# google/yggdrasil-decision-forests

Hardware: NVIDIA H100
Metric: GBT boosting iters/sec, 10M rows x 200 num feats (higher is better)
Workload: dtype int64 fixed-point sums (q24 gradients), f64 split scores

## Files before the change

include/ygg_b200.h:

```cpp
#ifndef YGG_B200_H_
#define YGG_B200_H_

#include <stdint.h>

#ifdef __cplusplus
extern "C" {
#endif

#define YGG_ABI_VERSION 3

enum ygg_status {
  YGG_OK = 0,
  YGG_ERR_INVALID_ARGUMENT = 1,
  YGG_ERR_NO_DEVICE = 2,
  YGG_ERR_CUDA = 3,
  YGG_ERR_UNIMPLEMENTED = 4,
  YGG_ERR_CANCELLED = 5,
  YGG_ERR_IO = 6
};

enum ygg_loss {
  YGG_LOSS_BINOMIAL_LOG_LIKELIHOOD = 0,
  YGG_LOSS_SQUARED_ERROR = 1,
  YGG_LOSS_MULTINOMIAL_LOG_LIKELIHOOD = 2
// ... 145 lines not shown
int ygg_gbt_tie_stats(ygg_gbt* h, int64_t* renamed, int64_t* unresolved);
int ygg_gbt_set_tie_rng_position(ygg_gbt* h, uint64_t words);

int ygg_num_candidate_attributes(int32_t num_features, int32_t loss, int32_t num_candidate_attributes,
                                 float num_candidate_attributes_ratio, int32_t* k);
uint64_t ygg_candidate_key(uint32_t random_seed, int32_t tree, int32_t node, int32_t feature);
int ygg_gbt_set_candidate_sampling(ygg_gbt* h, int32_t num_candidate_attributes, float num_candidate_attributes_ratio);

int ygg_gbt_set_dart(ygg_gbt* h, float dropout_rate);
int ygg_gbt_get_dart_weights(ygg_gbt* h, float* out, int32_t capacity, int32_t* n);
int ygg_gbt_get_dart_dropped(ygg_gbt* h, int32_t iter, int32_t* out, int32_t capacity, int32_t* n);

int ygg_gbt_get_tree(ygg_gbt* h, int32_t iter, ygg_node* out, int32_t capacity, int32_t* n_nodes);
int ygg_gbt_get_category_set(ygg_gbt* h, int32_t iter, int32_t node, uint32_t* words, int32_t capacity, int32_t* n_words);
int ygg_gbt_train_loss(ygg_gbt* h, int32_t iter, float* loss, float* secondary);
int ygg_gbt_get_predictions(ygg_gbt* h, float* out, int64_t n);
int ygg_gbt_predict(ygg_gbt* h, const ygg_dataset* ds, float* out, int64_t n);

int ygg_gbt_set_predictions(ygg_gbt* h, const float* pred, int64_t n);

int ygg_tree_train_on_gradients(ygg_gbt* h, const float* gradients, const float* hessians,
                                ygg_node* out, int32_t capacity, int32_t* n_nodes);

enum ygg_hist_mode {
  YGG_HIST_ROOT_SUM = 0,
  YGG_HIST_PACKED = 1,
  YGG_HIST_SHARED = 2,
  YGG_HIST_HIST2 = 3,
  YGG_HIST_SEGMENTED = 4,
};
typedef struct ygg_hist_plan {
  int32_t mode;
  int32_t group;
  int32_t hist2_tiles;
  int32_t chunk_blocks;
  int32_t slot_window;
  int32_t grid;
} ygg_hist_plan;
int ygg_debug_hist_plan(const ygg_gbt* h, int32_t level, ygg_hist_plan* out);
int ygg_debug_level_histogram(ygg_gbt* h, int32_t level, const ygg_hist_plan* plan, const float* gradients,
                              const float* second, const int32_t* slot_of_row, int32_t n_slots, uint64_t* out_sum,
                              uint32_t* out_cnt, uint64_t* out_second, float* out_scales);

int ygg_debug_wide_histogram(ygg_gbt* h, int32_t n_slots, uint64_t* out_sum, uint32_t* out_cnt, uint64_t* out_second);

int ygg_debug_capture_candidates(ygg_gbt* h, int32_t enabled);
typedef struct ygg_level_node {
  int32_t node;
  int32_t candidate;
  int32_t derived;
  int32_t reserved;
  int64_t num_examples;
} ygg_level_node;
typedef struct ygg_candidate {
  int32_t found;
  float score;
  int32_t threshold_bin;
  int32_t lo, hi;
  int32_t num_pos_examples;
  float threshold_value;
  uint32_t cat_mask[8];
} ygg_candidate;
int ygg_debug_level_candidates(ygg_gbt* h, int32_t level, int32_t capacity, ygg_level_node* nodes, ygg_candidate* cands,
                               uint32_t* sets, int32_t set_words, int32_t* n_nodes, float* scales);
int ygg_debug_level_tried(ygg_gbt* h, int32_t level, int32_t capacity, uint8_t* tried, int32_t* first_node, int32_t* n_nodes);

int ygg_partition_rows(ygg_dataset* ds, const uint32_t* rows_in, int64_t n, int32_t feature,
// ... 14 lines not shown
```

yggdrasil-decision-forests_b200/_capi.py:

```python
import ctypes as C
import os

import numpy as np

from . import _build

_LIB = None


class YggError(RuntimeError):
    def __init__(self, code, msg):
        super().__init__(f"[ygg status {code}] {msg}")
        self.code = code


class GbtConfig(C.Structure):
    _fields_ = [
        ("abi_version", C.c_int32), ("loss", C.c_int32), ("num_trees", C.c_int32),
        ("shrinkage", C.c_float), ("max_depth", C.c_int32), ("min_examples", C.c_int32),
        ("in_split_min_examples_check", C.c_int32), ("use_hessian_gain", C.c_int32),
        ("l1_regularization", C.c_float), ("l2_regularization", C.c_float),
        ("l2_regularization_categorical", C.c_float), ("clamp_leaf_logit", C.c_float),
        ("hessian_split_score_subtract_parent", C.c_int32), ("random_seed", C.c_uint32),
        ("subsample", C.c_float), ("validation_ratio", C.c_float),
        ("sibling_subtraction", C.c_int32), ("early_stopping", C.c_int32),
        ("early_stopping_num_trees_look_ahead", C.c_int32), ("early_stopping_initial_iteration", C.c_int32),
        ("num_classes", C.c_int32), ("candidate_shuffle", C.c_int32), ("rng_words_consumed", C.c_uint32),
        ("split_jobs_draw_seeds", C.c_int32), ("growing_strategy", C.c_int32), ("max_num_nodes", C.c_int32),
        ("goss_alpha", C.c_float), ("goss_beta", C.c_float),
    ]


NODE_DTYPE = np.dtype([
    ("feature", "<i4"), ("threshold_bin", "<i4"), ("na_value", "<i4"), ("depth", "<i4"),
    ("neg_child", "<i4"), ("pos_child", "<i4"), ("split_score", "<f4"), ("leaf_value", "<f4"),
    ("num_examples", "<i8"), ("num_pos_examples", "<i8"), ("stat", "<f8", (3,)),
    ("condition_type", "<i4"), ("threshold_value", "<f4"), ("cat_mask", "<u4", (8,)),
])
assert NODE_DTYPE.itemsize == 112

FEATURE_DISCRETIZED_NUMERICAL = 0
FEATURE_CATEGORICAL = 1
FEATURE_NUMERICAL = 2

LEVEL_NODE_DTYPE = np.dtype([("node", "<i4"), ("candidate", "<i4"), ("derived", "<i4"), ("reserved", "<i4"),
                             ("num_examples", "<i8")])
assert LEVEL_NODE_DTYPE.itemsize == 24
CANDIDATE_DTYPE = np.dtype([("found", "<i4"), ("score", "<f4"), ("threshold_bin", "<i4"), ("lo", "<i4"), ("hi", "<i4"),
                            ("num_pos_examples", "<i4"), ("threshold_value", "<f4"), ("cat_mask", "<u4", (8,))])
assert CANDIDATE_DTYPE.itemsize == 60

HIST_ROOT_SUM, HIST_PACKED, HIST_SHARED, HIST2, HIST_SEGMENTED = 0, 1, 2, 3, 4


class HistPlan(C.Structure):
    _fields_ = [("mode", C.c_int32), ("group", C.c_int32), ("hist2_tiles", C.c_int32), ("chunk_blocks", C.c_int32),
                ("slot_window", C.c_int32), ("grid", C.c_int32)]

    def __repr__(self):
        return "HistPlan(%s)" % ", ".join("%s=%d" % (k, getattr(self, k)) for k, _ in self._fields_)

ALLGATHER_FN = C.CFUNCTYPE(C.c_int, C.c_void_p, C.c_void_p, C.c_void_p, C.c_int64, C.c_void_p)
ALLREDUCE_FN = C.CFUNCTYPE(C.c_int, C.c_void_p, C.c_void_p, C.c_int64, C.c_int32, C.c_int32, C.c_void_p)
REDUCESCATTER_FN = C.CFUNCTYPE(C.c_int, C.c_void_p, C.c_void_p, C.c_int64, C.c_int32, C.c_int32, C.c_void_p)

EXPORTS = [
    "ygg_abi_version", "ygg_last_error", "ygg_device_count", "ygg_dataset_create",
    "ygg_dataset_set_feature_types", "ygg_dataset_destroy", "ygg_dataset_num_rows", "ygg_dataset_num_features",
    "ygg_gbt_config_init", "ygg_gbt_create", "ygg_gbt_destroy", "ygg_gbt_set_labels_i32",
    "ygg_gbt_set_labels_f32", "ygg_gbt_set_weights_f32", "ygg_gbt_set_validation_weights_f32", "ygg_gbt_set_feature_shard", "ygg_gbt_set_row_shard", "ygg_gbt_set_row_shard_scatter", "ygg_feature_shard",
    "ygg_merge_shard_best", "ygg_gbt_initial_prediction",
    "ygg_gbt_train", "ygg_gbt_train_timed", "ygg_gbt_step", "ygg_gbt_sync", "ygg_gbt_num_trees", "ygg_gbt_get_tree",
    "ygg_gbt_train_loss", "ygg_gbt_get_predictions", "ygg_gbt_set_predictions", "ygg_gbt_predict",
    "ygg_tree_train_on_gradients", "ygg_debug_hist_plan", "ygg_debug_level_histogram", "ygg_partition_rows",
    "ygg_gbt_set_profiling", "ygg_gbt_get_profile", "ygg_gbt_save_ydf",
    "ygg_discretize_boundaries", "ygg_discretize_encode", "ygg_model_write_ydf",
    "ygg_validation_split_mask", "ygg_dataset_split_rows", "ygg_gbt_set_validation_i32",
    "ygg_gbt_set_validation_f32", "ygg_gbt_validation_loss", "ygg_gbt_num_iterations", "ygg_gbt_final_validation",
    "ygg_gen_discretized_boundaries", "ygg_dataset_builder_create", "ygg_dataset_builder_add_numerical",
    "ygg_dataset_builder_add_numerical_async", "ygg_dataset_builder_get_numerical",
    "ygg_dataset_builder_add_bins", "ygg_dataset_builder_finish", "ygg_dataset_builder_destroy",
    "ygg_dataset_get_bins", "ygg_dataset_set_bucket_values", "ygg_gbt_tie_stats", "ygg_gbt_set_tie_rng_position",
    "ygg_gbt_best_split_window_bytes", "ygg_gbt_set_best_split_window", "ygg_comm_window_create",
    "ygg_comm_unique_id", "ygg_comm_create", "ygg_comm_destroy", "ygg_comm_allreduce", "ygg_comm_allgather", "ygg_comm_reducescatter",
    "ygg_dataset_set_wide_column", "ygg_dataset_get_wide_column", "ygg_debug_wide_histogram",
    "ygg_dataset_set_wide_categorical_column", "ygg_gbt_get_category_set",
    "ygg_dataset_set_numerical_column", "ygg_dataset_get_numerical_column",
    "ygg_debug_capture_candidates", "ygg_debug_level_candidates",
    "ygg_num_candidate_attributes", "ygg_candidate_key", "ygg_gbt_set_candidate_sampling", "ygg_debug_level_tried",
    "ygg_gbt_set_dart", "ygg_gbt_get_dart_weights", "ygg_gbt_get_dart_dropped",
# ... 692 lines not shown
```

yggdrasil-decision-forests_b200/csrc/ygg_engine.cu:

```cuda
#include <algorithm>
#include <mutex>
#include <random>
#include <cmath>
#include <cstdarg>
#include <cstdio>
#include <cstdlib>
#include <cstring>
#include <limits>
#include <map>
#include <queue>
#include <string>
#include <thread>
#include <vector>

#include <cuda_runtime.h>
#include <cub/device/device_radix_sort.cuh>
#include <cub/device/device_scan.cuh>
#include <nvtx3/nvToolsExt.h>

#include "../../include/ygg_b200.h"
#include "ygg_internal.h"
#include "../../include/ygg_b200_model.h"
#include "ygg_kernels.cuh"
#include "ygg_wide.cuh"
#include "ygg_presort.cuh"
#include "ygg_hist_seg.cuh"

using namespace ygg;

namespace {

thread_local std::string g_last_error;

int set_error(int code, const char* fmt, ...) {
  char buf[1024];
  va_list ap;
  va_start(ap, fmt);
  vsnprintf(buf, sizeof(buf), fmt, ap);
  va_end(ap);
  g_last_error = buf;
  return code;
}

}

int ygg_set_error_msg(int code, const char* msg) { return set_error(code, "%s", msg); }

namespace {

#define YGG_CUDA(expr)                                                                          \
  do {                                                                                          \
    cudaError_t _e = (expr);                                                                    \
    if (_e != cudaSuccess)                                                                      \
      return set_error(YGG_ERR_CUDA, "%s failed: %s (%s:%d)", #expr, cudaGetErrorString(_e),    \
                       __FILE__, __LINE__);                                                     \
  } while (0)

#define YGG_RETURN_IF_ERROR(expr) \
// ... 29 lines not shown
  return YGG_OK;
}
template <typename T>
int dev_alloc_plain(T** p, size_t count) {
  YGG_CUDA(cudaMalloc(reinterpret_cast<void**>(p), std::max<size_t>(count, 1) * sizeof(T)));
  return YGG_OK;
}
inline void dev_free(void* p) {
  if (p != nullptr) cudaFreeAsync(p, nullptr);
}

struct ProfileSlot {
  double ms = 0;
  int64_t launches = 0;
};

}


struct LossRec {
  double loss_sum;
  unsigned long long correct;
};

enum ShardMode { kShardNone = 0, kShardFeatures = 1, kShardRows = 2 };

struct HistLaunch {
  int mode;
  int G, S;
  int chunk, grid;
  int window, passes;
  int FL, T;
  int SL;
};

struct ygg_gbt {
  ygg_dataset* ds = nullptr;
  ygg_gbt_config cfg{};
  cudaStream_t stream = nullptr;
  bool has_labels = false;
  uint8_t* d_label_u8 = nullptr;
  float* d_label_f32 = nullptr;
  float initial_prediction = 0.f;
  float* d_pred = nullptr;
  float* d_g = nullptr;
  float* d_h = nullptr;
  uint32_t* d_q24 = nullptr;
  uint32_t* d_hq24 = nullptr;
  uint2* d_act = nullptr;
  uint32_t* d_act_h = nullptr;
  int32_t* d_act_count = nullptr;
  int32_t* d_act_sub = nullptr;
  uint32_t* d_root_cnt = nullptr;
  bool root_cnt_valid = false;
  int n_blocks = 0;
  uint16_t* d_node_of_row = nullptr;
  DeviceState* d_st = nullptr;
  LevelDesc* d_levels = nullptr;
  Family* d_fam[2] = {nullptr, nullptr};
  int32_t* d_slot_node[2] = {nullptr, nullptr};
  NodeRec* d_nodes_all = nullptr;
  NodeRec* d_nodes_scratch = nullptr;
  int tree_capacity = 0;
  unsigned long long* d_hist_sum[2] = {nullptr, nullptr};
  uint32_t* d_hist_cnt[2] = {nullptr, nullptr};
  unsigned long long* d_hist_hsum[2] = {nullptr, nullptr};
// ... 309 lines not shown
  YGG_CUDA(cudaMemcpy(out_max, d_max, sizeof(uint32_t), cudaMemcpyDeviceToHost));
  return YGG_OK;
}

int raise_hist_smem_caps_once(int device) {
  static std::mutex mu;
  static std::vector<char> done;
  std::lock_guard<std::mutex> lock(mu);
  if (static_cast<int>(done.size()) <= device) done.resize(device + 1, 0);
  if (done[device]) return YGG_OK;
  size_t budget = 0;
  YGG_RETURN_IF_ERROR(hist_smem_budget(device, &budget));
  auto set_cap = [](size_t bytes) {
    return [bytes](auto kern) -> int {
      YGG_CUDA(cudaFuncSetAttribute(kern, cudaFuncAttributeMaxDynamicSharedMemorySize, static_cast<int>(bytes)));
      return YGG_OK;
    };
  };
  for (const bool hess : {false, true})
    for (const int mode : {kHistRootSum, kHistPacked, kHistShared})
      for (const bool multi : {false, true}) YGG_RETURN_IF_ERROR(for_hist_kernel(hess, mode, set_cap(budget), multi));
  const auto cap2 = set_cap(kHist2SmemBudget);
  YGG_RETURN_IF_ERROR(cap2(k_hist2<32, true>)); YGG_RETURN_IF_ERROR(cap2(k_hist2<32, false>));
  YGG_RETURN_IF_ERROR(cap2(k_hist2<16, true>)); YGG_RETURN_IF_ERROR(cap2(k_hist2<16, false>));
  YGG_RETURN_IF_ERROR(cap2(k_hist2<8, true>)); YGG_RETURN_IF_ERROR(cap2(k_hist2<8, false>));
  YGG_RETURN_IF_ERROR(set_cap(seg_smem_bytes(64))(k_hist_seg<32, 2>));
  YGG_RETURN_IF_ERROR(set_cap(seg_smem_bytes(32))(k_hist_seg<32, 1>));
  YGG_RETURN_IF_ERROR(set_cap(seg_smem_bytes(16))(k_hist_seg<16, 1>));
  YGG_RETURN_IF_ERROR(set_cap(seg_smem_bytes(8))(k_hist_seg<8, 1>));
  YGG_CUDA(cudaFuncSetAttribute(k_hist_seg<32, 2>, cudaFuncAttributePreferredSharedMemoryCarveout, cudaSharedmemCarveoutMaxShared));
  YGG_CUDA(cudaFuncSetAttribute(k_hist_seg<32, 1>, cudaFuncAttributePreferredSharedMemoryCarveout, cudaSharedmemCarveoutMaxShared));
  YGG_CUDA(cudaFuncSetAttribute(k_hist_seg<16, 1>, cudaFuncAttributePreferredSharedMemoryCarveout, cudaSharedmemCarveoutMaxShared));
  YGG_CUDA(cudaFuncSetAttribute(k_hist_seg<8, 1>, cudaFuncAttributePreferredSharedMemoryCarveout, cudaSharedmemCarveoutMaxShared));
  done[device] = 1;
  return YGG_OK;
}

int configure_launches(ygg_gbt* h) {
  (void)cudaGetLastError();
  const bool hh = hist_hess(h);
  size_t budget = 0;
  YGG_RETURN_IF_ERROR(hist_smem_budget(h->ds->device, &budget));
  YGG_RETURN_IF_ERROR(raise_hist_smem_caps_once(h->ds->device));
  const int f_count = h->hist_f_end - h->hist_f_begin;
  const int n_blocks = static_cast<int>(h->ds->n_pad / kBlockRows);
  const int kSubBlocks = sub_blocks_of(h);
  const double min_items = 1.0, min_items2 = 0.9;
  auto choose_chunk = [&](int n_fgroups, int grid, int step, double need) {
    const int max_c = std::max(step, kHistMaxChunkBlocks / step * step);
    const int min_chunks = std::max(1, (n_blocks + max_c - 1) / max_c);
    int best = max_c;
    double best_score = -1;
    for (int nc = min_chunks; nc <= std::max(min_chunks, n_blocks); nc++) {
      const int c = std::min(max_c, ((n_blocks + nc - 1) / nc + step - 1) / step * step);
      const int real_nc = (n_blocks + c - 1) / c;
      const double per_cta = static_cast<double>(real_nc) * n_fgroups / grid;
      if (per_cta > 8.0 && nc > min_chunks) break;
      const double fill = static_cast<double>(n_blocks) / (static_cast<double>(real_nc) * c);
      const double eff = per_cta / std::ceil(per_cta) * fill;
      const double score = eff + (per_cta >= need ? 0.08 : 0.0);
      if (score > best_score + 1e-9) { best_score = score; best = c; }
    }
    return best;
  };
  const int g_begin = h->hist_f_begin / 4, n_groups = (h->hist_f_end + 3) / 4 - g_begin;
  const char* env_hist2 = std::getenv("YGG_HIST2");
// ... 2 lines not shown
  for (int l = 0; l < h->num_levels; l++) {
    HistLaunch& pl = h->hist_plan[l];
    pl.mode = hh ? kHistShared : (l == 0 && !sampling(h)) ? kHistRootSum : kHistPacked;
    int S = level_slot_bound(h, l);
    pl.window = 0;
    pl.passes = 1;
    if (hist_smem_bytes(1, S, hh, pl.mode) > budget) {
      if (S > 254)
        return set_error(YGG_ERR_UNIMPLEMENTED, "max_depth=%d needs %d histogram slots at level %d; the active lists carry 8-bit slots",
                         h->cfg.max_depth, S, l);
      int s_pass = 1;
      while (hist_smem_bytes(1, 2 * s_pass + 1, hh, pl.mode) <= budget) s_pass *= 2;
      pl.window = s_pass;
      pl.passes = (S + s_pass - 1) / s_pass;
      S = s_pass + 1;
    }
    int G = 1;
    while (G < 8 && G < f_count && hist_smem_bytes(G + 1, S, hh, pl.mode) <= budget) G++;
    pl.G = G;
    pl.S = S;
    pl.grid = h->ds->num_sms;
    pl.FL = pl.T = 0;
    if (want_hist2 && !hh && S <= 2 && (l > 0 || pl.mode == kHistRootSum)) {
      int FL = 32;
      while (FL > 8 && FL / 2 >= 4 * n_groups) FL /= 2;
      int T = 2;
      if (hist2_smem_bytes(FL, S, T, l == 0) > kHist2SmemBudget) T = 1;
      if (hist2_smem_bytes(FL, S, T, l == 0) <= kHist2SmemBudget) { pl.FL = FL; pl.T = T; }
    }
    const bool packed = pl.mode == kHistPacked || (pl.FL > 0 && l > 0);
    const int n_fgroups = pl.FL > 0 ? (n_groups + pl.FL / 4 - 1) / (pl.FL / 4) : (f_count + G - 1) / G;
    pl.chunk = choose_chunk(n_fgroups, pl.grid, packed ? kSubBlocks : 1, pl.FL > 0 ? min_items2 : min_items);
    pl.SL = 0;
    khist_plan[l] = pl;
    const int S_level = level_slot_bound(h, l);
    if (!hh && l > 0 && pl.mode == kHistPacked && pl.FL == 0 && S_level >= seg_min_slots(f_count, h->ds->n)) {
      int SL = 32;
      while (SL > 8 && SL / 2 >= f_count) SL /= 2;
      pl.SL = SL;
      pl.G = 1;
      pl.S = S_level;
      pl.window = 0;
      pl.passes = 1;
      pl.grid = h->ds->num_sms * kSegMinBlocks;
      pl.chunk = std::min(std::max(kSubBlocks, kHistMaxChunkBlocks / kSubBlocks * kSubBlocks),
                          (n_blocks + kSubBlocks - 1) / kSubBlocks * kSubBlocks);
    }
  }
  {
    std::map<int, uint32_t> max_of_chunk;
    uint32_t* d_sub = nullptr;
    int status = YGG_OK;
    for (int l = 0; l < h->num_levels && status == YGG_OK; l++) {
      HistLaunch& pl = h->hist_plan[l];
      if (pl.mode != kHistPacked && (pl.FL == 0 || l == 0)) continue;
      int chunk = pl.chunk;
      while (chunk >= kSubBlocks) {
        auto it = max_of_chunk.find(chunk);
        if (it == max_of_chunk.end()) {
          uint32_t m = 0;
          status = chunk_max_count(h, chunk, &d_sub, &m);
          if (status != YGG_OK) break;
          it = max_of_chunk.emplace(chunk, m).first;
        }
        if (it->second <= kPackedMaxUpdates) break;
        const int smaller = static_cast<int>(static_cast<double>(chunk) * 0.9 * kPackedMaxUpdates / it->second) / kSubBlocks * kSubBlocks;
        const int next = std::min(smaller, chunk - kSubBlocks);
        chunk = (next < kSubBlocks && chunk > kSubBlocks) ? kSubBlocks : next;
      }
      if (chunk < kSubBlocks) {
        if (pl.SL > 0) pl = khist_plan[l];
        pl.mode = kHistShared;
        pl.FL = 0;
        pl.chunk = choose_chunk((f_count + pl.G - 1) / pl.G, pl.grid, 1, min_items);
      } else {
        pl.chunk = chunk;
      }
    }
    dev_free(d_sub);
    if (status != YGG_OK) return status;
  }
  h->part_smem_children = static_cast<int>((32 * 1024) / (kPartWords * sizeof(uint32_t)));
  return YGG_OK;
}

int allocate_wide_buffers(ygg_gbt* h) {
  const ygg_dataset* ds = h->ds;
  dev_free(h->d_wsum); dev_free(h->d_wcnt); dev_free(h->d_whsum);
  h->d_wsum = nullptr; h->d_wcnt = nullptr; h->d_whsum = nullptr;
  for (int i = 0; i < 2; i++) {
    dev_free(h->d_wnode_sum[i]); dev_free(h->d_wnode_cnt[i]); dev_free(h->d_wnode_hsum[i]);
    h->d_wnode_sum[i] = nullptr; h->d_wnode_cnt[i] = nullptr; h->d_wnode_hsum[i] = nullptr;
  }
  dev_free(h->d_wide_thr); dev_free(h->d_wide_feature); dev_free(h->d_wide_bins);
  h->d_wide_thr = nullptr; h->d_wide_feature = nullptr; h->d_wide_bins = nullptr;
  dev_free(h->d_wide_cat); dev_free(h->d_wide_na_bin); dev_free(h->d_wide_set); dev_free(h->d_sort_key); dev_free(h->d_sort_idx);
  h->d_wide_cat = nullptr; h->d_wide_na_bin = nullptr; h->d_wide_set = nullptr; h->d_sort_key = nullptr; h->d_sort_idx = nullptr;
  dev_free(h->d_sort_off); h->d_sort_off = nullptr;
  h->sort_total = 0;
  h->wide_total = 0;
  h->wide_slots = 0;
  if ((ds->n_wide() == 0 && ds->n_num() == 0) || h->num_levels == 0) return YGG_OK;
  YGG_CUDA(cudaDeviceSynchronize());
  const int f_scan = h->f_end - h->f_begin;
  const size_t nodes = static_cast<size_t>(1) << std::max(0, h->num_levels - 1);
  YGG_RETURN_IF_ERROR(dev_alloc(&h->d_wide_thr, nodes * f_scan));
  if (ds->n_wide() == 0) return YGG_OK;
  h->wide_total = ds->wide_off.back();
  h->wide_slots = level_slot_bound(h, h->num_levels - 1);
  const bool hh = hist_hess(h);
  const size_t per_bucket = sizeof(unsigned long long) + sizeof(uint32_t) + (hh ? sizeof(unsigned long long) : 0);
  const size_t slot_elems = static_cast<size_t>(h->wide_slots) * h->wide_total, node_elems = nodes * h->wide_total;
  auto fail = [&]() {
// ... 293 lines not shown
  YGG_RETURN_IF_ERROR(ensure_seg_buffers(h));
  const int f_count = h->hist_f_end - h->hist_f_begin;
  const int n_chunks = (h->n_blocks + pl.chunk - 1) / pl.chunk;
  const int fpl = seg_lane_features(pl.SL, f_count);
  const int n_fg = seg_feature_groups(pl.SL, fpl, h->hist_f_begin, f_count);
  const int target_pieces = std::max(1, (kSegItemsPerCta * pl.grid + n_fg - 1) / n_fg);
  k_seg_count<<<std::min(h->n_blocks, ds->num_sms * 8), 256, 0, h->stream>>>(h->d_act, h->d_act_count, h->n_blocks, pl.S,
                                                                               levels, l, h->d_hseg_blk);
  YGG_RETURN_IF_ERROR(check_launch("k_seg_count"));
  YGG_CUDA(cub::DeviceScan::InclusiveSum(h->d_hseg_temp, h->hseg_temp_bytes, h->d_hseg_blk, h->d_hseg_blk, pl.S * h->n_blocks,
                                         h->stream));
  k_seg_ranges<<<1, kSegScanThreads, 0, h->stream>>>(h->d_hseg_blk, pl.S, h->n_blocks, pl.chunk, n_chunks, target_pieces,
                                                     h->d_hseg_off, h->d_hseg_piece, h->d_hseg_meta);
  YGG_RETURN_IF_ERROR(check_launch("k_seg_ranges"));
  k_seg_scatter<<<std::min(h->n_blocks, ds->num_sms * 8), 256, 0, h->stream>>>(h->d_act, h->d_act_count, h->n_blocks, pl.S, levels, l,
                                                               h->d_hseg_blk, h->d_hseg);
  YGG_RETURN_IF_ERROR(check_launch("k_seg_scatter"));
  SegParams sp{};
  sp.rows = ds->d_bins_rows; sp.row_bytes = static_cast<uint32_t>(seg_row_bytes(ds->F));
  sp.seg = h->d_hseg; sp.seg_off = h->d_hseg_off; sp.piece_start = h->d_hseg_piece; sp.meta = h->d_hseg_meta;
  sp.n_ranges = pl.S * n_chunks; sp.n_chunks = n_chunks;
  sp.f_begin = h->hist_f_begin; sp.f_count = f_count;
  sp.hist_sum = lb.sum; sp.hist_cnt = lb.cnt;
  sp.f_chunk = lb.f_chunk; sp.chunk_stride = static_cast<long long>(lb.chunk_u64);
  const size_t smem = seg_smem_bytes(pl.SL * fpl);
  if (fpl == 2) k_hist_seg<32, 2><<<pl.grid, kSegThreads, smem, h->stream>>>(sp);
  else if (pl.SL == 32) k_hist_seg<32, 1><<<pl.grid, kSegThreads, smem, h->stream>>>(sp);
  else if (pl.SL == 16) k_hist_seg<16, 1><<<pl.grid, kSegThreads, smem, h->stream>>>(sp);
  else k_hist_seg<8, 1><<<pl.grid, kSegThreads, smem, h->stream>>>(sp);
  h->launches_total += 5;
  return check_launch("k_hist_seg");
}

int ensure_root_counts(ygg_gbt* h) {
  if (h->root_cnt_valid) return YGG_OK;
  const int f_count = h->hist_f_end - h->hist_f_begin;
  if (h->d_root_cnt) dev_free(h->d_root_cnt);
  h->d_root_cnt = nullptr;
  const LevelBuf lb = level_buf(h, 1, 1);
  const size_t padded = static_cast<size_t>(lb.W) * lb.f_chunk * kMaxBins;
  YGG_RETURN_IF_ERROR(dev_alloc(&h->d_root_cnt, padded));
  YGG_CUDA(cudaMemsetAsync(h->d_root_cnt, 0, padded * sizeof(uint32_t), h->stream));
  dim3 grid(std::max(1, h->ds->num_sms * 8 / std::max(1, f_count)), f_count);
  k_root_counts<<<grid, 256, 0, h->stream>>>(h->ds->d_bins, h->ds->n, h->ds->n_pad, f_count, h->hist_f_begin, h->d_root_cnt);
  h->launches_total++;
  YGG_RETURN_IF_ERROR(check_launch("k_root_counts"));
  h->root_cnt_valid = true;
  return YGG_OK;
}

int accumulate_level(ygg_gbt* h, int l, const LevelBuf& lb, const LevelDesc* levels, const HistLaunch& pl) {
  const ygg_dataset* ds = h->ds;
  const int hist_f_count = h->hist_f_end - h->hist_f_begin;
  YGG_RETURN_IF_ERROR(zero_planes(h, lb));
  if (pl.mode == kHistRootSum) {
    const size_t row = static_cast<size_t>(lb.f_chunk) * kMaxBins * sizeof(uint32_t);
    YGG_CUDA(cudaMemcpy2DAsync(lb.cnt, lb.chunk_u64 * sizeof(unsigned long long), h->d_root_cnt, row, row, lb.W,
                               cudaMemcpyDeviceToDevice, h->stream));
  }
  if (pl.SL > 0) return launch_hist_seg(h, l, lb, levels, pl);
  if (pl.FL > 0) {
    YGG_RETURN_IF_ERROR(ensure_bins4(h->ds));
    Hist2Params hp{};
    hp.bins4 = ds->d_bins4; hp.n_pad = ds->n_pad; hp.n = ds->n; hp.q24 = h->d_q24; hp.act = h->d_act;
    hp.act_count = h->d_act_count; hp.act_sub = h->d_act_sub; hp.n_blocks = h->n_blocks;
    hp.f_begin = h->hist_f_begin; hp.f_count = hist_f_count;
    hp.g_begin = h->hist_f_begin / 4; hp.n_groups = (h->hist_f_end + 3) / 4 - hp.g_begin;
    hp.S = pl.S; hp.T = pl.T; hp.chunk_blocks = pl.chunk;
    hp.level = l; hp.levels = levels;
    hp.hist_sum = lb.sum; hp.hist_cnt = lb.cnt;
    hp.f_chunk = lb.f_chunk; hp.chunk_stride = static_cast<long long>(lb.chunk_u64);
    return launch_hist2(h, hp, pl.FL, l == 0, pl.grid);
  }
  HistParams hp{};
  hp.bins = ds->d_bins; hp.n_pad = ds->n_pad; hp.act = h->d_act; hp.act_h = h->d_act_h; hp.q24 = h->d_q24;
  hp.act_count = h->d_act_count; hp.n_blocks = h->n_blocks;
  hp.f_begin = h->hist_f_begin; hp.f_count = hist_f_count; hp.G = pl.G; hp.S = pl.S;
  hp.chunk_blocks = pl.chunk;
  hp.level = l; hp.levels = levels;
  hp.hist_sum = lb.sum; hp.hist_cnt = lb.cnt; hp.hist_hsum = lb.hsum;
  hp.f_chunk = lb.f_chunk; hp.chunk_stride = static_cast<long long>(lb.chunk_u64);
  const size_t smem = hist_smem_bytes(pl.G, pl.S, hist_hess(h), pl.mode);
  if (pl.window > 0) {
    for (int pass = 0; pass < pl.passes; pass++) {
      hp.level = l | ((pass * pl.window) << 8) | (pl.window << 20);
      YGG_RETURN_IF_ERROR(launch_hist(h, hp, pl.mode, pl.grid, smem, true));
    }
    return YGG_OK;
  }
  return launch_hist(h, hp, pl.mode, pl.grid, smem);
}

int do_allreduce(ygg_gbt* h, void* buf, int64_t count, int dtype, int op) {
// ... 2360 lines not shown
  YGG_CUDA(cudaMemcpyAsync(h->d_g, gradients, n * sizeof(float), cudaMemcpyHostToDevice, h->stream));
  if (has_h(h)) YGG_CUDA(cudaMemcpyAsync(h->d_h, hessians, n * sizeof(float), cudaMemcpyHostToDevice, h->stream));
  const int root_candidate = (n >= h->cfg.min_examples && 1 < h->cfg.max_depth) ? 1 : 0;
  k_begin_iteration<<<1, 1, 0, h->stream>>>(h->d_st, h->d_levels, h->d_fam[0], h->d_slot_node[0], root_candidate);
  h->launches_total++;
  k_absmax<<<elementwise_grid(h), 256, 0, h->stream>>>(h->d_g, n, h->d_st);
  h->launches_total++;
  YGG_RETURN_IF_ERROR(check_launch("k_absmax"));
  h->scratch_tree = false;
  YGG_RETURN_IF_ERROR(grow_tree(h, h->d_nodes_scratch));
  if (h->cfg.growing_strategy == 1) YGG_RETURN_IF_ERROR(best_first_prune(h, h->d_nodes_scratch));
  YGG_RETURN_IF_ERROR(check_device_error(h));
  h->scratch_tree = true;
  std::vector<ygg_node> flat;
  YGG_RETURN_IF_ERROR(fetch_tree(h, h->d_nodes_scratch, &flat, true));
  *n_nodes = static_cast<int32_t>(flat.size());
  if (static_cast<int32_t>(flat.size()) > capacity) return set_error(YGG_ERR_INVALID_ARGUMENT, "capacity %d < %zu nodes", capacity, flat.size());
  std::memcpy(out, flat.data(), flat.size() * sizeof(ygg_node));
  return YGG_OK;
}

int ygg_debug_hist_plan(const ygg_gbt* h, int32_t level, ygg_hist_plan* out) {
  if (!h || !out) return set_error(YGG_ERR_INVALID_ARGUMENT, "null argument");
  if (level < 0 || level >= h->num_levels) return set_error(YGG_ERR_INVALID_ARGUMENT, "level %d outside [0, %d)", level, h->num_levels);
  const HistLaunch& pl = h->hist_plan[level];
  ygg_hist_plan p{};
  if (pl.FL > 0) {
    p.mode = YGG_HIST_HIST2; p.group = pl.FL; p.hist2_tiles = pl.T;
  } else if (pl.SL > 0) {
    p.mode = YGG_HIST_SEGMENTED; p.group = pl.SL;
  } else {
    p.mode = pl.mode == kHistRootSum ? YGG_HIST_ROOT_SUM : pl.mode == kHistPacked ? YGG_HIST_PACKED : YGG_HIST_SHARED;
    p.group = pl.G;
  }
  p.chunk_blocks = pl.chunk;
  p.slot_window = pl.window;
  p.grid = pl.grid;
  *out = p;
  return YGG_OK;
}

int ygg_debug_level_histogram(ygg_gbt* h, int32_t level, const ygg_hist_plan* plan, const float* gradients,
                              const float* second, const int32_t* slot_of_row, int32_t n_slots, uint64_t* out_sum,
                              uint32_t* out_cnt, uint64_t* out_second, float* out_scales) {
  if (!h || !gradients || !slot_of_row || !out_sum || !out_cnt || !out_scales) return set_error(YGG_ERR_INVALID_ARGUMENT, "null argument");
  if (level < 0 || level >= h->num_levels) return set_error(YGG_ERR_INVALID_ARGUMENT, "level %d outside [0, %d)", level, h->num_levels);
  if (n_slots < 1 || n_slots > 254) return set_error(YGG_ERR_INVALID_ARGUMENT, "n_slots=%d outside [1, 254] (8-bit slots)", n_slots);
  const bool hh = hist_hess(h);
  if (hh != (second != nullptr) || hh != (out_second != nullptr))
    return set_error(YGG_ERR_INVALID_ARGUMENT, hh ? "this handle keeps a second histogram plane: `second` and `out_second` are required"
                                                  : "this handle keeps no second histogram plane: `second` and `out_second` must be NULL");
  const float v_pow2 = hh ? (weighted(h) ? h->w_pow2 : h_pow2_of(h)) : 0.f;
  const int64_t n = h->ds->n;
  bool all_slot0 = true;
  for (int64_t r = 0; r < n; r++) {
    if (!std::isfinite(gradients[r])) return set_error(YGG_ERR_INVALID_ARGUMENT, "gradient of row %lld is not finite", static_cast<long long>(r));
    if (hh && !(second[r] >= 0.f && second[r] <= v_pow2))
      return set_error(YGG_ERR_INVALID_ARGUMENT, "second-plane value of row %lld outside [0, %g]", static_cast<long long>(r), v_pow2);
    if (slot_of_row[r] < -1 || slot_of_row[r] >= n_slots)
      return set_error(YGG_ERR_INVALID_ARGUMENT, "slot %d of row %lld outside [-1, %d)", slot_of_row[r], static_cast<long long>(r), n_slots);
    all_slot0 &= slot_of_row[r] == 0;
  }
  HistLaunch pl{};
  if (plan == nullptr) {
    pl = h->hist_plan[level];
    if (n_slots > level_slot_bound(h, level))
      return set_error(YGG_ERR_INVALID_ARGUMENT, "the plan of level %d holds %d slots, %d requested", level, level_slot_bound(h, level), n_slots);
  } else {
    const ygg_hist_plan& p = *plan;
    if (p.mode < YGG_HIST_ROOT_SUM || p.mode > YGG_HIST_SEGMENTED) return set_error(YGG_ERR_INVALID_ARGUMENT, "unknown mode %d", p.mode);
    if (p.chunk_blocks < 1 || p.chunk_blocks > kHistMaxChunkBlocks)
      return set_error(YGG_ERR_INVALID_ARGUMENT, "chunk_blocks=%d outside [1, %d]", p.chunk_blocks, kHistMaxChunkBlocks);
    if (p.grid < 1 || p.grid > 65535) return set_error(YGG_ERR_INVALID_ARGUMENT, "grid=%d outside [1, 65535]", p.grid);
    if (p.slot_window < 0) return set_error(YGG_ERR_INVALID_ARGUMENT, "slot_window=%d", p.slot_window);
    pl.chunk = p.chunk_blocks; pl.grid = p.grid;
    if (p.mode == YGG_HIST_HIST2) {
      if (p.group != 8 && p.group != 16 && p.group != 32) return set_error(YGG_ERR_INVALID_ARGUMENT, "k_hist2: %d feature lanes (8, 16 or 32)", p.group);
      if (p.hist2_tiles != 1 && p.hist2_tiles != 2) return set_error(YGG_ERR_INVALID_ARGUMENT, "k_hist2: %d sub-tiles (1 or 2)", p.hist2_tiles);
      if (p.slot_window != 0) return set_error(YGG_ERR_INVALID_ARGUMENT, "k_hist2 has no multi-pass form");
      if (n_slots > 2) return set_error(YGG_ERR_INVALID_ARGUMENT, "k_hist2 with %d slots (at most 2)", n_slots);
      if (hist2_smem_bytes(p.group, n_slots, p.hist2_tiles, level == 0) > kHist2SmemBudget)
        return set_error(YGG_ERR_INVALID_ARGUMENT, "k_hist2 needs %zu bytes of shared memory (budget 216 KB)", hist2_smem_bytes(p.group, n_slots, p.hist2_tiles, level == 0));
      pl.FL = p.group; pl.T = p.hist2_tiles; pl.S = n_slots; pl.G = 1; pl.passes = 1;
      pl.mode = level == 0 ? kHistRootSum : kHistPacked;
    } else if (p.mode == YGG_HIST_SEGMENTED) {
      if (level == 0) return set_error(YGG_ERR_INVALID_ARGUMENT, "k_hist_seg runs below the root only");
      if (hh) return set_error(YGG_ERR_INVALID_ARGUMENT, "a second histogram plane is accumulated by the shared layout only");
      if (p.group != 8 && p.group != 16 && p.group != 32) return set_error(YGG_ERR_INVALID_ARGUMENT, "k_hist_seg: %d feature lanes (8, 16 or 32)", p.group);
      if (p.slot_window != 0) return set_error(YGG_ERR_INVALID_ARGUMENT, "k_hist_seg has no multi-pass form");
      pl.SL = p.group; pl.S = n_slots; pl.G = 1; pl.passes = 1;
      pl.mode = kHistPacked;
    } else {
      if (p.group < 1 || p.group > 8) return set_error(YGG_ERR_INVALID_ARGUMENT, "k_hist: group=%d outside [1, 8]", p.group);
      pl.mode = p.mode == YGG_HIST_ROOT_SUM ? kHistRootSum : p.mode == YGG_HIST_PACKED ? kHistPacked : kHistShared;
      pl.G = p.group;
      if (p.slot_window > 0) {
        if (pl.mode == kHistRootSum) return set_error(YGG_ERR_INVALID_ARGUMENT, "the root layout has no multi-pass form");
        pl.window = p.slot_window; pl.S = p.slot_window + 1; pl.passes = (n_slots + p.slot_window - 1) / p.slot_window;
      } else {
        pl.S = n_slots; pl.passes = 1;
      }
      size_t budget = 0;
      YGG_RETURN_IF_ERROR(hist_smem_budget(h->ds->device, &budget));
      if (hist_smem_bytes(pl.G, pl.S, hh, pl.mode) > budget)
        return set_error(YGG_ERR_INVALID_ARGUMENT, "k_hist with G=%d and %d slots per pass needs %zu bytes of shared memory (budget %zu)",
                         pl.G, pl.S, hist_smem_bytes(pl.G, pl.S, hh, pl.mode), budget);
    }
  }
  if (hh && (pl.FL > 0 || pl.SL > 0 || pl.mode != kHistShared))
    return set_error(YGG_ERR_INVALID_ARGUMENT, "a second histogram plane is accumulated by the shared layout only");
  if (pl.mode == kHistRootSum && (level != 0 || sampling(h) || !all_slot0 || n_slots != 1))
    return set_error(YGG_ERR_INVALID_ARGUMENT, "the root layouts need level 0, no row sampling and every row in slot 0");
  if (h->wide_total > 0 && n_slots > h->wide_slots)
    return set_error(YGG_ERR_INVALID_ARGUMENT, "the wide-column planes of this handle hold %d slots, %d requested", h->wide_slots, n_slots);
  YGG_CUDA(cudaSetDevice(h->ds->device));
  (void)cudaGetLastError();
  if (pl.mode == kHistPacked) {
    const int sub = sub_blocks_of(h);
    if (pl.chunk % sub != 0)
      return set_error(YGG_ERR_INVALID_ARGUMENT, "packed layout: chunk_blocks=%d is not a multiple of the %d-block sub-chunk", pl.chunk, sub);
    uint32_t* d_sub = nullptr;
    uint32_t m = 0;
    const int st = chunk_max_count(h, pl.chunk, &d_sub, &m);
    dev_free(d_sub);
    YGG_RETURN_IF_ERROR(st);
    if (m > kPackedMaxUpdates)
      return set_error(YGG_ERR_INVALID_ARGUMENT, "packed layout: a bin receives %u rows in one chunk of %d blocks (at most %u)", m, pl.chunk, kPackedMaxUpdates);
  }
  if (pl.mode == kHistRootSum) YGG_RETURN_IF_ERROR(ensure_root_counts(h));
  YGG_RETURN_IF_ERROR(raise_hist_smem_caps_once(h->ds->device));

  const int64_t n_pad = h->ds->n_pad;
  const int f_hist = h->hist_f_end - h->hist_f_begin;
  std::vector<uint8_t> sel(n), slot8(n);
  for (int64_t r = 0; r < n; r++) {
    sel[r] = slot_of_row[r] >= 0 ? 1 : 0;
    slot8[r] = static_cast<uint8_t>(slot_of_row[r] >= 0 ? slot_of_row[r] : 0);
  }
  std::vector<LevelDesc> lv(32, LevelDesc{0, 0, 0, 0});
  lv[level] = LevelDesc{0, n_slots, n_slots, 0};
  const LevelBuf probe = level_buf(h, n_slots, 1);
  float *d_g = nullptr, *d_v = nullptr;
// ... 506 lines not shown
```

yggdrasil-decision-forests_b200/csrc/ygg_hist_seg.cuh:

```cuda
#pragma once
#include <cstdint>
#include <type_traits>
#include <cub/block/block_scan.cuh>
#include <cuda_runtime.h>

#include "ygg_device.cuh"
#include "ygg_hist.cuh"

namespace ygg {

constexpr int kSegThreads = 1024;
constexpr int kSegMinBlocks = 1;
constexpr int kSegMinSlots = 4;
constexpr int kSegShallowMinFeatures = 128;
constexpr long long kSegShallowMinElements = 1000000000LL;
constexpr int kSegItemsPerCta = 4;
constexpr int kSegMinPiece = 4096;
constexpr int kSegMaxSlots = 256;
constexpr int kSegScanThreads = 512;

inline int seg_lane_features(int FL, int f_count) { return FL == 32 && f_count > 32 ? 2 : 1; }
inline int seg_min_slots(int f_count, long long rows) {
  return f_count >= kSegShallowMinFeatures && rows * f_count >= kSegShallowMinElements ? 1 : kSegMinSlots;
}
__host__ __device__ inline size_t seg_smem_bytes(int FI) { return static_cast<size_t>(kMaxBins) * 2 * FI * 4; }
__host__ __device__ inline int seg_feature_groups(int FL, int FPL, int f_begin, int f_count) {
  const int off = FPL == 2 ? (f_begin & 1) : 0;
  return (f_count + off + FL * FPL - 1) / (FL * FPL);
}
inline int seg_row_bytes(int F) {
  int b = 32;
  while (b < F && b < 256) b *= 2;
  return b >= F ? b : (F + 255) / 256 * 256;
}

__global__ void __launch_bounds__(256) k_bins_to_rows(const uint8_t* bins, int64_t n_pad, int F, int row_bytes, uint8_t* rows) {
  const int64_t r = static_cast<int64_t>(blockIdx.x) * 256 + threadIdx.x;
  const int f0 = blockIdx.y * 32;
  if (r >= n_pad) return;
  uint32_t w[8] = {0u, 0u, 0u, 0u, 0u, 0u, 0u, 0u};
#pragma unroll
  for (int k = 0; k < 32; k++) {
    const int f = f0 + k;
    const uint32_t v = f < F ? bins[static_cast<int64_t>(f) * n_pad + r] : 0u;
    w[k >> 2] |= v << (8 * (k & 3));
  }
  uint4* dst = reinterpret_cast<uint4*>(rows + r * row_bytes + f0);
  dst[0] = make_uint4(w[0], w[1], w[2], w[3]);
  dst[1] = make_uint4(w[4], w[5], w[6], w[7]);
}

__device__ __forceinline__ uint32_t seg_slot_of(uint2 e, bool valid, uint32_t ns) {
  const uint32_t slot = e.x >> 24;
  return (valid && slot < ns) ? slot : 0xFFFFFFFFu;
}

__global__ void __launch_bounds__(256) k_seg_count(const uint2* act, const int32_t* act_count, int n_blocks, int S,
                                                   const LevelDesc* levels, int level, long long* blk) {
  __shared__ int c[kSegMaxSlots];
  const uint32_t ns = static_cast<uint32_t>(min(S, levels[level].num_slots));
// ... 231 lines not shown
```

Baseline: 163.3.

## Add row-major root histogram kernel with 32-bit shared sums and carry counters

Adds a new root-level histogram kernel that reads the row-major bin layout, which the segmented deeper levels already use. Each lane owns four features, accumulates 32-bit fixed-point sums in shared memory with 16-bit carry counters, then flushes 64-bit totals to global memory with atomics. It is enabled for level 0 when the deeper levels use the segmented kernel and the dataset is wide and large. The aim is to cut root histogram cost and share one bin layout across levels, at the price of extra carry handling and a larger shared-memory footprint.

```diff
diff --git a/include/ygg_b200.h b/include/ygg_b200.h
--- a/include/ygg_b200.h
+++ b/include/ygg_b200.h
@@ -201,7 +201,10 @@
 typedef struct ygg_hist_plan {
   int32_t mode;
   int32_t group;
-  int32_t hist2_tiles;
+  union {
+    int32_t hist2_tiles;
+    int32_t root_lanes;
+  };
   int32_t chunk_blocks;
   int32_t slot_window;
   int32_t grid;
diff --git a/yggdrasil-decision-forests_b200/_capi.py b/yggdrasil-decision-forests_b200/_capi.py
--- a/yggdrasil-decision-forests_b200/_capi.py
+++ b/yggdrasil-decision-forests_b200/_capi.py
@@ -56,6 +56,8 @@
 class HistPlan(C.Structure):
     _fields_ = [("mode", C.c_int32), ("group", C.c_int32), ("hist2_tiles", C.c_int32), ("chunk_blocks", C.c_int32),
                 ("slot_window", C.c_int32), ("grid", C.c_int32)]
+
+    root_lanes = property(lambda self: self.hist2_tiles, lambda self, v: setattr(self, "hist2_tiles", v))
 
     def __repr__(self):
         return "HistPlan(%s)" % ", ".join("%s=%d" % (k, getattr(self, k)) for k, _ in self._fields_)
diff --git a/yggdrasil-decision-forests_b200/csrc/ygg_engine.cu b/yggdrasil-decision-forests_b200/csrc/ygg_engine.cu
--- a/yggdrasil-decision-forests_b200/csrc/ygg_engine.cu
+++ b/yggdrasil-decision-forests_b200/csrc/ygg_engine.cu
@@ -24,6 +24,7 @@
 #include "ygg_kernels.cuh"
 #include "ygg_wide.cuh"
 #include "ygg_presort.cuh"
+#include "ygg_hist_root.cuh"
 #include "ygg_hist_seg.cuh"
 
 using namespace ygg;
@@ -119,6 +120,7 @@
   int window, passes;
   int FL, T;
   int SL;
+  int RL;
 };
 
 struct ygg_gbt {
@@ -494,6 +496,7 @@
   YGG_CUDA(cudaFuncSetAttribute(k_hist_seg<32, 1>, cudaFuncAttributePreferredSharedMemoryCarveout, cudaSharedmemCarveoutMaxShared));
   YGG_CUDA(cudaFuncSetAttribute(k_hist_seg<16, 1>, cudaFuncAttributePreferredSharedMemoryCarveout, cudaSharedmemCarveoutMaxShared));
   YGG_CUDA(cudaFuncSetAttribute(k_hist_seg<8, 1>, cudaFuncAttributePreferredSharedMemoryCarveout, cudaSharedmemCarveoutMaxShared));
+  YGG_RETURN_IF_ERROR(set_cap(kRootSmemBytes)(k_hist_root_rows));
   done[device] = 1;
   return YGG_OK;
 }
@@ -562,6 +565,7 @@
     const int n_fgroups = pl.FL > 0 ? (n_groups + pl.FL / 4 - 1) / (pl.FL / 4) : (f_count + G - 1) / G;
     pl.chunk = choose_chunk(n_fgroups, pl.grid, packed ? kSubBlocks : 1, pl.FL > 0 ? min_items2 : min_items);
     pl.SL = 0;
+    pl.RL = 0;
     khist_plan[l] = pl;
     const int S_level = level_slot_bound(h, l);
     if (!hh && l > 0 && pl.mode == kHistPacked && pl.FL == 0 && S_level >= seg_min_slots(f_count, h->ds->n)) {
@@ -609,6 +613,19 @@
     }
     dev_free(d_sub);
     if (status != YGG_OK) return status;
+  }
+  if (h->num_levels > 0 && h->hist_plan[0].mode == kHistRootSum && h->hist_plan[0].FL == 0 &&
+      seg_min_slots(f_count, h->ds->n) == 1) {
+    bool seg = false;
+    for (int l = 1; l < h->num_levels; l++) seg |= h->hist_plan[l].SL > 0;
+    if (seg) {
+      HistLaunch& pl = h->hist_plan[0];
+      pl.RL = kRootLanes;
+      pl.G = kRootFpl;
+      pl.S = 1;
+      pl.grid = h->ds->num_sms;
+      pl.chunk = choose_chunk(seg_feature_groups(kRootLanes, kRootFpl, h->hist_f_begin, f_count), pl.grid, 1, 0.0);
+    }
   }
   h->part_smem_children = static_cast<int>((32 * 1024) / (kPartWords * sizeof(uint32_t)));
   return YGG_OK;
@@ -968,6 +985,19 @@
   return check_launch("k_hist_seg");
 }
 
+int launch_hist_root_rows(ygg_gbt* h, const LevelBuf& lb, const HistLaunch& pl) {
+  ygg_dataset* ds = h->ds;
+  YGG_RETURN_IF_ERROR(ensure_bins_rows(ds));
+  RootRowsParams rp{};
+  rp.rows = ds->d_bins_rows; rp.row_bytes = static_cast<uint32_t>(seg_row_bytes(ds->F));
+  rp.q24 = h->d_q24; rp.act_count = h->d_act_count; rp.n_blocks = h->n_blocks; rp.chunk_blocks = pl.chunk;
+  rp.f_begin = h->hist_f_begin; rp.f_count = h->hist_f_end - h->hist_f_begin;
+  rp.hist_sum = lb.sum; rp.f_chunk = lb.f_chunk; rp.chunk_stride = static_cast<long long>(lb.chunk_u64);
+  k_hist_root_rows<<<pl.grid, kRootThreads, kRootSmemBytes, h->stream>>>(rp);
+  h->launches_total++;
+  return check_launch("k_hist_root_rows");
+}
+
 int ensure_root_counts(ygg_gbt* h) {
   if (h->root_cnt_valid) return YGG_OK;
   const int f_count = h->hist_f_end - h->hist_f_begin;
@@ -995,6 +1025,7 @@
                                cudaMemcpyDeviceToDevice, h->stream));
   }
   if (pl.SL > 0) return launch_hist_seg(h, l, lb, levels, pl);
+  if (pl.RL > 0) return launch_hist_root_rows(h, lb, pl);
   if (pl.FL > 0) {
     YGG_RETURN_IF_ERROR(ensure_bins4(h->ds));
     Hist2Params hp{};
@@ -3421,6 +3452,7 @@
   } else {
     p.mode = pl.mode == kHistRootSum ? YGG_HIST_ROOT_SUM : pl.mode == kHistPacked ? YGG_HIST_PACKED : YGG_HIST_SHARED;
     p.group = pl.G;
+    p.root_lanes = pl.RL;
   }
   p.chunk_blocks = pl.chunk;
   p.slot_window = pl.window;
@@ -3458,8 +3490,12 @@
   } else {
     const ygg_hist_plan& p = *plan;
     if (p.mode < YGG_HIST_ROOT_SUM || p.mode > YGG_HIST_SEGMENTED) return set_error(YGG_ERR_INVALID_ARGUMENT, "unknown mode %d", p.mode);
-    if (p.chunk_blocks < 1 || p.chunk_blocks > kHistMaxChunkBlocks)
-      return set_error(YGG_ERR_INVALID_ARGUMENT, "chunk_blocks=%d outside [1, %d]", p.chunk_blocks, kHistMaxChunkBlocks);
+    const bool root_rows = p.mode == YGG_HIST_ROOT_SUM && p.root_lanes != 0;
+    if (root_rows && p.root_lanes != kRootLanes)
+      return set_error(YGG_ERR_INVALID_ARGUMENT, "root_lanes=%d: 0 (k_hist) or %d (k_hist_root_rows)", p.root_lanes, kRootLanes);
+    const int max_chunk = root_rows ? kRootRowsMaxChunkBlocks : kHistMaxChunkBlocks;
+    if (p.chunk_blocks < 1 || p.chunk_blocks > max_chunk)
+      return set_error(YGG_ERR_INVALID_ARGUMENT, "chunk_blocks=%d outside [1, %d]", p.chunk_blocks, max_chunk);
     if (p.grid < 1 || p.grid > 65535) return set_error(YGG_ERR_INVALID_ARGUMENT, "grid=%d outside [1, 65535]", p.grid);
     if (p.slot_window < 0) return set_error(YGG_ERR_INVALID_ARGUMENT, "slot_window=%d", p.slot_window);
     pl.chunk = p.chunk_blocks; pl.grid = p.grid;
@@ -3479,6 +3515,11 @@
       if (p.slot_window != 0) return set_error(YGG_ERR_INVALID_ARGUMENT, "k_hist_seg has no multi-pass form");
       pl.SL = p.group; pl.S = n_slots; pl.G = 1; pl.passes = 1;
       pl.mode = kHistPacked;
+    } else if (root_rows) {
+      if (p.group != kRootFpl) return set_error(YGG_ERR_INVALID_ARGUMENT, "k_hist_root_rows: group=%d features per lane (%d)", p.group, kRootFpl);
+      if (p.slot_window != 0) return set_error(YGG_ERR_INVALID_ARGUMENT, "the root layout has no multi-pass form");
+      pl.RL = p.root_lanes; pl.G = p.group; pl.S = n_slots; pl.passes = 1;
+      pl.mode = kHistRootSum;
     } else {
       if (p.group < 1 || p.group > 8) return set_error(YGG_ERR_INVALID_ARGUMENT, "k_hist: group=%d outside [1, 8]", p.group);
       pl.mode = p.mode == YGG_HIST_ROOT_SUM ? kHistRootSum : p.mode == YGG_HIST_PACKED ? kHistPacked : kHistShared;
@@ -3496,7 +3537,7 @@
                          pl.G, pl.S, hist_smem_bytes(pl.G, pl.S, hh, pl.mode), budget);
     }
   }
-  if (hh && (pl.FL > 0 || pl.SL > 0 || pl.mode != kHistShared))
+  if (hh && (pl.FL > 0 || pl.SL > 0 || pl.RL > 0 || pl.mode != kHistShared))
     return set_error(YGG_ERR_INVALID_ARGUMENT, "a second histogram plane is accumulated by the shared layout only");
   if (pl.mode == kHistRootSum && (level != 0 || sampling(h) || !all_slot0 || n_slots != 1))
     return set_error(YGG_ERR_INVALID_ARGUMENT, "the root layouts need level 0, no row sampling and every row in slot 0");
diff --git a/yggdrasil-decision-forests_b200/csrc/ygg_hist_root.cuh b/yggdrasil-decision-forests_b200/csrc/ygg_hist_root.cuh
--- /dev/null
+++ b/yggdrasil-decision-forests_b200/csrc/ygg_hist_root.cuh
@@ -0,0 +1,149 @@
+#pragma once
+#include <cstdint>
+#include <cuda_runtime.h>
+
+#include "ygg_device.cuh"
+#include "ygg_hist.cuh"
+#include "ygg_hist_seg.cuh"
+
+namespace ygg {
+
+constexpr int kRootThreads = 1024;
+constexpr int kRootLanes = 32;
+constexpr int kRootFpl = 4;
+constexpr int kRootFeatures = kRootLanes * kRootFpl;
+constexpr int kRootRowsPerWarp = 8;
+constexpr int kRootRowsMaxChunkBlocks = 2048;
+static_assert(static_cast<unsigned long long>(kRootRowsMaxChunkBlocks) * kBlockRows * kQMax >> 32 < (1ull << 16),
+              "the 16-bit carry counters of a chunk");
+constexpr size_t kRootSmemBytes = static_cast<size_t>(kMaxBins) * kRootFeatures * (4 + 2);
+
+struct RootRowsParams {
+  const uint8_t* rows;
+  uint32_t row_bytes;
+  const uint32_t* q24;
+  const int32_t* act_count;
+  int n_blocks, chunk_blocks;
+  int f_begin, f_count;
+  unsigned long long* hist_sum;
+  int f_chunk;
+  long long chunk_stride;
+};
+
+__device__ __forceinline__ uint32_t ldg_row_word(const uint8_t* p) {
+  return __ldg(reinterpret_cast<const uint32_t*>(p));
+}
+
+__global__ void __launch_bounds__(kRootThreads, 1) k_hist_root_rows(RootRowsParams p) {
+  constexpr int kWarps = kRootThreads / 32;
+  constexpr int U = kRootRowsPerWarp;
+  constexpr uint32_t kSumWords = kMaxBins * kRootFeatures;
+  extern __shared__ __align__(16) uint32_t s_sum[];
+  uint32_t* s_carry = s_sum + kSumWords;
+  const int tid = threadIdx.x, lane = tid & 31, warp = tid >> 5;
+  uint32_t s_base = static_cast<uint32_t>(__cvta_generic_to_shared(s_sum));
+  asm volatile("mov.u32 %0, %0;" : "+r"(s_base));
+  const uint32_t a_lane = s_base + static_cast<uint32_t>(lane) * 4u;
+  const uint32_t c_lane = s_base + kSumWords * 4u + static_cast<uint32_t>(lane >> 1) * 4u;
+  const uint32_t c_inc = 1u << (16 * (lane & 1));
+  const int off = p.f_begin & (kRootFpl - 1);
+  const int n_fg = seg_feature_groups(kRootLanes, kRootFpl, p.f_begin, p.f_count);
+  const int n_chunks = (p.n_blocks + p.chunk_blocks - 1) / p.chunk_blocks;
+  const int n_items = n_chunks * n_fg;
+  for (int i = tid; i < static_cast<int>(kRootSmemBytes / 4); i += kRootThreads) s_sum[i] = 0u;
+  __syncthreads();
+
+  for (int item = blockIdx.x; item < n_items; item += gridDim.x) {
+    const int chunk = item / n_fg, fg = item - chunk * n_fg;
+    const int f0 = fg * kRootFeatures - off;
+    const int last = min(kRootFeatures, p.f_count - f0) - 1;
+    const uint8_t* col = p.rows + p.f_begin + f0 + min(lane * kRootFpl, last & ~(kRootFpl - 1));
+    const int64_t r0 = static_cast<int64_t>(chunk) * p.chunk_blocks * kBlockRows;
+    const int64_t r1 = min(static_cast<int64_t>(p.n_blocks), static_cast<int64_t>(chunk + 1) * p.chunk_blocks) * kBlockRows;
+
+    uint32_t w[U];
+    uint4 qv[U / 4];
+    int cnt = 0;
+    auto load = [&](int64_t r) {
+      if (r < r1) {
+#pragma unroll
+        for (int u = 0; u < U; u++) w[u] = ldg_row_word(col + static_cast<size_t>(r + u) * p.row_bytes);
+#pragma unroll
+        for (int v = 0; v < U / 4; v++) qv[v] = __ldg(reinterpret_cast<const uint4*>(p.q24 + r) + v);
+        cnt = __ldg(p.act_count + (r / kBlockRows));
+      }
+    };
+    int64_t r = r0 + static_cast<int64_t>(warp) * U;
+    load(r);
+    for (; r < r1; r += static_cast<int64_t>(kWarps) * U) {
+      uint32_t wc[U], q[U];
+#pragma unroll
+      for (int u = 0; u < U; u++) wc[u] = w[u];
+#pragma unroll
+      for (int v = 0; v < U / 4; v++) {
+        q[4 * v] = qv[v].x; q[4 * v + 1] = qv[v].y; q[4 * v + 2] = qv[v].z; q[4 * v + 3] = qv[v].w;
+      }
+      const int in_block = static_cast<int>(r & (kBlockRows - 1));
+#pragma unroll
+      for (int u = 0; u < U; u++) q[u] = in_block + u < cnt ? q[u] : 0u;
+      load(r + static_cast<int64_t>(kWarps) * U);
+#pragma unroll
+      for (int u = 0; u < U; u += 2) {
+        uint32_t a[2 * kRootFpl], old[2 * kRootFpl];
+#pragma unroll
+        for (int j = 0; j < 2; j++)
+#pragma unroll
+          for (int k = 0; k < kRootFpl; k++)
+            a[j * kRootFpl + k] = a_lane + static_cast<uint32_t>(k) * 128u + (((wc[u + j] >> (8 * k)) & 0xFFu) << 9);
+#pragma unroll
+        for (int j = 0; j < 2; j++)
+#pragma unroll
+          for (int k = 0; k < kRootFpl; k++) old[j * kRootFpl + k] = smem_add(a[j * kRootFpl + k], q[u + j]);
+        bool carry = false;
+#pragma unroll
+        for (int j = 0; j < 2; j++)
+#pragma unroll
+          for (int k = 0; k < kRootFpl; k++) carry |= old[j * kRootFpl + k] + q[u + j] < old[j * kRootFpl + k];
+        if (carry) {
+#pragma unroll
+          for (int j = 0; j < 2; j++)
+#pragma unroll
+            for (int k = 0; k < kRootFpl; k++)
+              if (old[j * kRootFpl + k] + q[u + j] < old[j * kRootFpl + k])
+                smem_red(c_lane + ((a[j * kRootFpl + k] - a_lane) >> 1), c_inc);
+        }
+      }
+    }
+    __syncthreads();
+
+    constexpr int TB = 8, QL = 4;
+    constexpr int kQuadGroups = kRootLanes / (4 * QL);
+    constexpr int kTiles = kMaxBins / TB * kRootFpl * kQuadGroups;
+    const int tr = lane / QL, tq = lane % QL;
+    for (int t = warp; t < kTiles; t += kWarps) {
+      const int bin = t / (kRootFpl * kQuadGroups) * TB + tr;
+      const int k = t / kQuadGroups % kRootFpl;
+      const int l0 = (t % kQuadGroups * QL + tq) * 4;
+      const int wi = (bin * kRootFpl + k) * kRootLanes + l0;
+      uint4* sw = reinterpret_cast<uint4*>(s_sum + wi);
+      uint2* cw = reinterpret_cast<uint2*>(s_carry + wi / 2);
+      const uint4 lo4 = *sw;
+      const uint2 c2 = *cw;
+      *sw = make_uint4(0u, 0u, 0u, 0u);
+      *cw = make_uint2(0u, 0u);
+      const uint32_t los[4] = {lo4.x, lo4.y, lo4.z, lo4.w};
+      const uint32_t cs[4] = {c2.x & 0xFFFFu, c2.x >> 16, c2.y & 0xFFFFu, c2.y >> 16};
+#pragma unroll
+      for (int j = 0; j < 4; j++) {
+        const int f = f0 + (l0 + j) * kRootFpl + k;
+        const unsigned long long sum = static_cast<unsigned long long>(cs[j]) << 32 | los[j];
+        if (sum == 0ull || f < 0 || f >= p.f_count) continue;
+        size_t oc;
+        atomicAdd(&p.hist_sum[slot_hist_offset(0, f, bin, p.f_chunk, p.chunk_stride, &oc)], sum);
+      }
+    }
+    __syncthreads();
+  }
+}
+
+}
diff --git a/yggdrasil-decision-forests_b200/csrc/ygg_hist_seg.cuh b/yggdrasil-decision-forests_b200/csrc/ygg_hist_seg.cuh
--- a/yggdrasil-decision-forests_b200/csrc/ygg_hist_seg.cuh
+++ b/yggdrasil-decision-forests_b200/csrc/ygg_hist_seg.cuh
@@ -25,7 +25,7 @@
 }
 __host__ __device__ inline size_t seg_smem_bytes(int FI) { return static_cast<size_t>(kMaxBins) * 2 * FI * 4; }
 __host__ __device__ inline int seg_feature_groups(int FL, int FPL, int f_begin, int f_count) {
-  const int off = FPL == 2 ? (f_begin & 1) : 0;
+  const int off = f_begin & (FPL - 1);
   return (f_count + off + FL * FPL - 1) / (FL * FPL);
 }
 inline int seg_row_bytes(int F) {
```

Measured after the change: 168.3, median of 6. 3.1% higher.
